# rogeliorjr/DyCON_Paper_Replication

Hardware: AMD Instinct MI355X
Metric: train volumes/sec (96^3 patch) (higher is better)
Workload: dtype bf16

## Files before the change

### dycon_paper_replication_amd/_lib.py

```python
from __future__ import annotations

import ctypes as C
import os

_HERE = os.path.dirname(os.path.abspath(__file__))
LIB_PATH = os.environ.get("DYCON_LIB", os.path.join(_HERE, "libdycon_hip.so"))

F32, BF16 = 0, 1
CONV_1X1, CONV_K3, CONV_K2S2 = 0, 1, 2

P, I, L, F, Z, U64 = C.c_void_p, C.c_int, C.c_longlong, C.c_float, C.c_size_t, C.c_uint64

SIGNATURES = {
    "dycon_version": (I, []),
    "dycon_last_error": (C.c_char_p, []),
    "dycon_bfrag_bytes": (Z, [I, I, I, I]),
    "dycon_pack_bfrag": (I, [P, P, I, I, I, I, I, L, L, L, L, I, P]),
    "dycon_pack_batch": (I, [P, I, I, P]),
    "dycon_pack_tcn": (I, [P, P, I, I, I, I, L, L, L, L, I, P]),
    "dycon_conv_gemm_workspace": (Z, [I, I, I, I, I, I, I, I, I]),
    "dycon_conv_gemm_plan": (I, [I, I, I, I, I, I, I, I, I, I, I, P]),
    "dycon_conv_kernel_name": (C.c_char_p, [I]),
    "dycon_conv_region_name": (C.c_char_p, [P]),
    "dycon_conv_gemm": (I, [P, P, P, P, I, I, I, I, I, I, I, I, I, I, I, P, Z, P]),
    "dycon_conv_gemm_splits": (I, [I, I, I, I, I, I, I, I, I]),
    "dycon_conv_gemm_ex": (I, [P, P, P, P, I, I, I, I, I, I, I, I, I, I, I, P, Z, I, P]),
    "dycon_conv_direct": (I, [P, I, P, P, P, I, I, I, I, I, I, I, I, I, P]),
    "dycon_conv_wgrad_workspace": (Z, [I, I, I, I, I, I, I]),
    "dycon_conv_wgrad_name": (C.c_char_p, [I, I, I, I, I, I, I, I, I]),
    "dycon_conv_wgrad": (I, [P, I, P, I, P, P, I, I, I, I, I, I, I, L, L, L, P, Z, P]),
    "dycon_colsum_workspace": (Z, [L, I]),
    "dycon_colsum": (I, [P, I, P, L, I, P, Z, P]),
    "dycon_norm_workspace": (Z, [I, L, I]),
    "dycon_norm_stats": (I, [P, I, I, L, I, I, F, P, P, P, F, P, Z, P]),
    "dycon_norm_fwd": (I, [P, P, I, I, L, I, I, F, P, P, P, I, P, P, P, P, F, P, Z, P]),
    "dycon_norm_fwd_is_fused": (I, [I, L, I, I]),
    "dycon_norm_fwd_slab": (I, [P, I, P, P, P, I, I, L, I, I, F, P, P, P, I, P, P, P]),
    "dycon_norm_apply": (I, [P, P, I, I, L, I, I, P, P, P, I, P, P, P]),
    "dycon_norm_bwd": (I, [P, I, P, P, I, I, L, I, I, P, P, P, I, P, P, P, P, Z, P]),
    "dycon_norm_bwd_ex": (I, [P, I, P, P, I, I, L, I, I, P, P, P, I, P, P, P, I, P, Z, P]),
    "dycon_norm_sum_dparams": (I, [P, I, I, P, P, P]),
# ... 243 lines not shown
```

### dycon_paper_replication_amd/csrc/conv.hip

```cpp
#include <stdlib.h>

#include "common.h"

typedef float f32x4 __attribute__((ext_vector_type(4)));
typedef __bf16 bf16x8 __attribute__((ext_vector_type(8)));

template <typename T> struct Frag;
template <> struct Frag<float> { static constexpr int G = 4, KC = 16; };
template <> struct Frag<bf16> { static constexpr int G = 8, KC = 32; };

__device__ __forceinline__ void mma(f32x4& acc, const Vec16<float>& a, const Vec16<float>& b) {
    acc = __builtin_amdgcn_mfma_f32_16x16x4f32(a.v.x, b.v.x, acc, 0, 0, 0);
    acc = __builtin_amdgcn_mfma_f32_16x16x4f32(a.v.y, b.v.y, acc, 0, 0, 0);
    acc = __builtin_amdgcn_mfma_f32_16x16x4f32(a.v.z, b.v.z, acc, 0, 0, 0);
    acc = __builtin_amdgcn_mfma_f32_16x16x4f32(a.v.w, b.v.w, acc, 0, 0, 0);
}
__device__ __forceinline__ void mma(f32x4& acc, const Vec16<bf16>& a, const Vec16<bf16>& b) {
    acc = __builtin_amdgcn_mfma_f32_16x16x32_bf16(__builtin_bit_cast(bf16x8, a.v), __builtin_bit_cast(bf16x8, b.v),
                                                  acc, 0, 0, 0);
}

template <int MODE> __device__ __forceinline__ int n_taps() { return MODE == DYCON_CONV_K3 ? 27 : MODE == DYCON_CONV_K2S2 ? 8 : 1; }

template <int MODE>
// ... 86 lines not shown
            if (++c == jb.Cin) { c = 0; ++t; }
        }
        if (jb.kind == 0) {
            uint4 o;
            o.x = (unsigned)f32_to_bf16_bits(v[0]) | ((unsigned)f32_to_bf16_bits(v[1]) << 16);
            o.y = (unsigned)f32_to_bf16_bits(v[2]) | ((unsigned)f32_to_bf16_bits(v[3]) << 16);
            o.z = (unsigned)f32_to_bf16_bits(v[4]) | ((unsigned)f32_to_bf16_bits(v[5]) << 16);
            o.w = (unsigned)f32_to_bf16_bits(v[6]) | ((unsigned)f32_to_bf16_bits(v[7]) << 16);
            reinterpret_cast<uint4*>(jb.out)[pi] = o;
        } else {
            reinterpret_cast<float4*>(jb.out)[pi] = make_float4(v[0], v[1], v[2], v[3]);
        }
    }
}

constexpr int NTB = 4;

template <typename T, int MODE, bool SCATTER>
__global__ __launch_bounds__(256) void conv_gemm_kernel(const T* __restrict__ X, const T* __restrict__ Wf,
                                                        const float* __restrict__ bias, T* __restrict__ Y, int B, int Di,
                                                        int Hi, int Wi, int Cin, int Do, int Ho, int Wo, int N, int Cout,
                                                        int NT, int nKC, int accumulate, float* __restrict__ slab,
                                                        int kc_per_split, int span_major = 0) {
    constexpr int G = Frag<T>::G, KC = Frag<T>::KC;
    const int lane = threadIdx.x & 63, wave = threadIdx.x >> 6;
    const int r = lane & 15, kg = lane >> 4;
    const long long M = (long long)B * Do * Ho * Wo;
    const long long m = (long long)blockIdx.x * 64 + wave * 16 + r;
    const bool mvalid = m < M;
    int xo, yo, zo, bo;
    {
        long long q = mvalid ? m : 0;
// ... 89 lines not shown
                                 2 * ox + (tap & 1);
            off = ov * Cout + co;
        } else {
            off = mo * N + n0;
        }
        Vec16<T> o = ld16(Ot + row * OS + pc * VN);
        if (accumulate) {
            const Vec16<T> old = ld16(Y + off);
#pragma unroll
            for (int k = 0; k < VN; ++k) o.set(k, o.get(k) + old.get(k));
        }
        st16(Y + off, o);
    }
}

constexpr int CT_BM = 64, CT_BN = 128, CT_AS = 40;
constexpr int CT_OS = CT_BN + 4;

template <int KS2>
__global__ __launch_bounds__(256, KS2 == 1 ? 4 : 3) void conv_k3_tile_kernel(const bf16* __restrict__ X, const bf16* __restrict__ Wf,
                                                           const float* __restrict__ bias, bf16* __restrict__ Y,
                                                           float* __restrict__ slab, int B, int D, int H, int W, int Cin, int N,
                                                           int NT, int nKC, int kc_per_split, int accumulate, int span_major = 0) {
    constexpr int A_ELEMS = CT_BM * CT_AS, B_ELEMS = 8 * 64 * 8;
    constexpr int KLOOP_BYTES = 2 * KS2 * (A_ELEMS + B_ELEMS) * 2, EPI_BYTES = CT_BM * CT_OS * 4;
    __shared__ __attribute__((aligned(16))) unsigned char lds_raw[KLOOP_BYTES > EPI_BYTES ? KLOOP_BYTES : EPI_BYTES];
    unsigned short (*As)[KS2][A_ELEMS] = reinterpret_cast<unsigned short (*)[KS2][A_ELEMS]>(lds_raw);
    unsigned short (*Bs)[KS2][B_ELEMS] = reinterpret_cast<unsigned short (*)[KS2][B_ELEMS]>(lds_raw + 2 * KS2 * A_ELEMS * 2);
    const int lane = threadIdx.x & 63, wave = threadIdx.x >> 6;
    const int r = lane & 15, kg = lane >> 4;
    const int wm = wave >> 1, wn = wave & 1;
// ... 172 lines not shown
            const int hz = hv / 36, hy = (hv / 6) % 6, hx = hv % 6;
            const int zi = z0 + hz - 1, yi = y0 + hy - 1, xi = x0 + hx - 1;
            v[i] = make_uint4(0, 0, 0, 0);
            if (p < PIECES && (unsigned)zi < (unsigned)D && (unsigned)yi < (unsigned)H && (unsigned)xi < (unsigned)W)
                v[i] = *reinterpret_cast<const uint4*>(xb + (((long long)zi * H + yi) * W + xi) * CH_CIN + sl * 8);
        }
#pragma unroll
        for (int i = 0; i < PER; ++i) {
            const int p = tid + i * 64 * CH_NW, hv = p >> 4, sl = p & 15;
            const int hy = (hv / 6) % 6, hx = hv % 6;
            if (p < PIECES) *reinterpret_cast<uint4*>(lds + hv * 256 + ((sl ^ (4 * (hy & 3) + (hx & 3))) * 16)) = v[i];
        }
    }

    auto load_b = [&](int kc, uint4 (&bf)[NJ]) {
        const uint4* p = reinterpret_cast<const uint4*>(Wf + ((long long)kc * NT + nt0 + cg * NJ) * 512) + lane;
#pragma unroll
        for (int j = 0; j < NJ; ++j) bf[j] = p[j * 64];
    };
    f32x4 acc[4][NJ];
#pragma unroll
    for (int m = 0; m < 4; ++m)
#pragma unroll
        for (int j = 0; j < NJ; ++j) acc[m][j] = f32x4{0.f, 0.f, 0.f, 0.f};
    auto compute = [&](int kc, const uint4 (&bf)[NJ]) {
        const int t = kc >> 2, kq = kc & 3;
        const int dz = t / 9, dy = (t / 3) % 3, dx = t % 3;
        const int hy = ry + dy, hx = rx + dx;
        const int slot = (4 * kq + kg) ^ (4 * (hy & 3) + (hx & 3));
        const unsigned char* ap = lds + ((dz * CH_H + hy) * CH_H + hx) * 256 + slot * 16;
        bf16x8 a[4];
// ... 2091 lines not shown
        pack_bfrag_kernel<T><<<grid, 256, 0, stream>>>(w, (T*)out, Tn, Cin, N, N0, s_t, s_c, s_n1, s_n0, flip_taps, NT, total);
    });
    DYCON_LAUNCH_CHECK();
    return DYCON_OK;
}

extern "C" int dycon_pack_tcn(const float* w, float* out, int T, int Cin, int N, int N0, long long s_t, long long s_c,
                              long long s_n1, long long s_n0, int flip_taps, dycon_stream_t stream) {
    DYCON_REQUIRE(w && out && T > 0 && Cin > 0 && N > 0 && N0 > 0, "pack_tcn: bad arguments");
    const long long total = (long long)T * Cin * N;
    pack_tcn_kernel<<<cdiv(total, 256), 256, 0, stream>>>(w, out, T, Cin, N, N0, s_t, s_c, s_n1, s_n0, flip_taps, total);
    DYCON_LAUNCH_CHECK();
    return DYCON_OK;
}

struct SplitK { int splits, kc_per_split; };
static SplitK splitk_plan(int dtype, int mode, int scatter, long long M, int N, int Cin) {
    const int KC = dtype == DYCON_BF16 ? 32 : 16;
    const int Tn = mode == DYCON_CONV_K3 ? 27 : mode == DYCON_CONV_K2S2 ? 8 : 1;
    const int nKC = (Tn * Cin + KC - 1) / KC;
    const long long wgs = ((M + 63) / 64) * (((N + 15) / 16 + NTB - 1) / NTB);
    SplitK p{1, nKC};
    if (scatter || wgs >= 512 || nKC < 16) return p;
    long long s = (1024 + wgs - 1) / wgs;
    if (s > nKC / 6) s = nKC / 6;
    if (s < 2) return p;
    p.kc_per_split = (int)((nKC + s - 1) / s);
    p.splits = (nKC + p.kc_per_split - 1) / p.kc_per_split;
    return p;
}
static SplitK conv_tile_plan(long long M, int N, int Cin) {
    constexpr long long target_wgs = 512;
    const int nKC = 27 * Cin / 32;
    const long long wgs = ((M + CT_BM - 1) / CT_BM) * (N / CT_BN);
    SplitK p{1, nKC};
    if (wgs >= 384) return p;
    long long s = target_wgs / wgs;
    if (s > nKC / 8) s = nKC / 8;
    if (s < 2) return p;
    p.kc_per_split = (int)((nKC + s - 1) / s);
    if (Cin % 64 == 0) p.kc_per_split = (p.kc_per_split + 1) & ~1;
    p.splits = (nKC + p.kc_per_split - 1) / p.kc_per_split;
    return p;
}

constexpr long long CONV_LDS_MIN_VOXELS = 13824;
static bool conv_first_layer(int dtype, int mode, int scatter, int Di, int Hi, int Wi, int Cin, int Cout) {
    return dtype == DYCON_BF16 && mode == DYCON_CONV_K3 && !scatter && Cin == 1 && (Cout == 16 || Cout == 32 || Cout == 64) &&
           (long long)Di * Hi * Wi >= CONV_LDS_MIN_VOXELS;
}
struct ConvRefusal { const char* fmt; int arg; };
static ConvRefusal conv_refusal(int dtype, int mode, int scatter, int B, int Di, int Hi, int Wi, int Cin, int N, int Cout) {
    if (!(B > 0 && Di > 0 && Hi > 0 && Wi > 0 && Cin > 0 && N > 0 && Cout > 0)) return {"conv_gemm: bad shape", 0};
    if (mode < 0 || mode > 2) return {"conv_gemm: bad mode %d", mode};
    if (!conv_first_layer(dtype, mode, scatter, Di, Hi, Wi, Cin, Cout) && Cin % (dtype == DYCON_BF16 ? 8 : 4) != 0)
        return {"conv_gemm: Cin=%d not a multiple of the fragment width", Cin};
    if (N % 16 != 0) return {"conv_gemm: N=%d not a multiple of 16 (use dycon_conv_direct)", N};
    if (scatter && !(mode == DYCON_CONV_1X1 && N == 8 * Cout)) return {"conv_gemm: scatter needs mode 1x1 and N == 8*Cout", 0};
    if (!scatter && N != Cout) return {"conv_gemm: N must equal Cout without scatter", 0};
// ... 559 lines not shown
```

### dycon_paper_replication_amd/engine.py

```python
from __future__ import annotations

from collections import OrderedDict
from typing import Dict, Optional

import torch

from . import ops
from ._lib import CONV_1X1, CONV_C1, CONV_K2S2, CONV_K3, CONV_W_CHUNK16

UNET_FILTERS = (16, 32, 64, 128, 256)
VNET_NORMS = ("groupnorm", "instancenorm", "batchnorm", "none")


def _projection_spec(spec, c_in):
    spec["projection.0.weight"] = (512, c_in, 1, 1, 1)
    spec["projection.0.bias"] = (512,)
    spec["projection.1.weight"] = (512,)
    spec["projection.1.bias"] = (512,)
    spec["projection.3.weight"] = (256, 512, 1, 1, 1)
    spec["projection.3.bias"] = (256,)
    spec["projection.4.weight"] = (256,)
    spec["projection.4.bias"] = (256,)


# ... 147 lines not shown
        self.use_aspp = net_type == "unet_3D" and "aspp.conv1.weight" in params
        self._aspp_plans = {}
        self._jobs_split, self._pack_event = False, None
        self.on_param_grads = None
        self.wgrad_stream = None
        self.wgrad_stream2 = None
        self._wg_flip = 0
        self.feat_stream = None
        self.mark = None
        self.Gs = {}
        self._head_range = (0, 0)
        self._wws = {}
        self.fuse_finish = False
        self.conv_stats = False
        self.conv_stats96 = False
        self._stat_parts = {}
        self._deferred = {}
        self._pending_dparams = []
        self.tape = []
        self.G = {}

    def params_changed(self):
        self.gen += 1

    def _pk(self, key, kind, w, T, Cin, N, N0, s_t, s_c, s_n1, s_n0, flip=False):
        hit = self._packed.get(key)
        if hit is not None and hit[0] == self.gen:
            return hit[1]
        buf = hit[1] if hit is not None else None
        if kind == "frag":
            buf = ops.pack_bfrag(w, self.dtype, T, Cin, N, N0, s_t, s_c, s_n1, s_n0, flip, out=buf)
            code = 0 if self.dtype == torch.bfloat16 else 1
# ... 94 lines not shown
    def _peek(self, t):
        g = self.G.get(id(t))
        if g is not None:
            self._sync_to(id(t), g)
        return g

    def _put(self, t, g):
        self.G[id(t)] = g
        if self.feat_stream is not None:
            self.Gs[id(t)] = ops.cur_stream()

    def _give(self, t, g):
        cur = self._peek(t)
        self._put(t, g if cur is None else ops.add(cur, g))

    def _conv(self, name, x, kind, need_gx=True, out_dtype=None, norm_groups=0):
        w, b = self.p[name + ".weight"], self.p[name + ".bias"]
        dtype = self.dtype
        if kind == "deconv":
            Cin, Cout = w.shape[0], w.shape[1]
        else:
            Cout, Cin = w.shape[0], w.shape[1]
        T = {"k3": 27, "k2s2": 8, "deconv": 8, "1x1": 1}[kind]
        mode = {"k3": CONV_K3, "k2s2": CONV_K2S2, "deconv": CONV_1X1, "1x1": CONV_1X1}[kind]
        gq = 8 if dtype == torch.bfloat16 else 4
        skinny = (Cin % gq != 0) or (Cout % 16 != 0)
        out_dtype = out_dtype or dtype
        plan = ops.conv_plan_for(x, mode, Cout, Cout) if kind == "k3" and out_dtype == dtype else None
        first_lds = plan is not None and plan.family == CONV_C1

        def conv_with_stats(wf, want):
# ... 11 lines not shown
                y = ops.conv_gemm(x, wf, b, CONV_K3, Cout, Cout)
        elif skinny:
            assert kind in ("k3", "1x1"), "skinny path only for the first conv and the 1x1 heads"
            wt = self._pk((name, "tcn"), "tcn", w, T, Cin, Cout, Cout, 1, T, 0, Cin * T)
            y = ops.conv_direct(x, wt, b, mode, Cout, out_dtype)
        elif kind == "deconv":
            wf = self._pk((name, "f"), "frag", w, 1, Cin, 8 * Cout, Cout, 0, Cout * 8, 1, 8)
            y = ops.conv_gemm(x, wf, b, CONV_1X1, 8 * Cout, Cout, scatter=True)
        elif plan is not None and plan.weights == CONV_W_CHUNK16:
            wf = self._pk_chunked16((name, "f48"), w, 3, Cout, 1, 27, Cin * 27)
            y = ops.conv_gemm(x, wf, b, mode, Cout, Cout)
        else:
            wf = self._pk((name, "f"), "frag", w, T, Cin, Cout, Cout, 1, T, 0, Cin * T)
            Vo = (x.shape[1] * x.shape[2] * x.shape[3]) // (8 if kind == "k2s2" else 1)
            want_stats = self.conv_stats96 if (Cin, Cout) == (16, 16) else self.conv_stats
            y = conv_with_stats(wf, want_stats and kind == "k3" and out_dtype == dtype and dtype == torch.bfloat16)
            if y is None and (norm_groups and self.fuse_finish and dtype == torch.bfloat16 and out_dtype == dtype
                              and ops.norm_fwd_is_fused(x, Vo, Cout, norm_groups)):
                y, dc = ops.conv_gemm(x, wf, b, mode, Cout, Cout, defer_finish=True)
                if dc is not None:
                    self._deferred[id(y)] = dc
            elif y is None:
                y = ops.conv_gemm(x, wf, b, mode, Cout, Cout)

        if self.recording:
            def wgrad(gy):
                gw, gb = self.g[name + ".weight"], self.g[name + ".bias"]
                wkey = (name, tuple(x.shape[:4]))
                ws = self._wws.get(wkey)
                if kind == "deconv":
                    if ws is None:
# ... 89 lines not shown
            if self.recording:
                def bwd_relu():
                    gy = self._take(y)
                    if skip is not None:
                        self._give(skip, gy)
                    self._give(z, ops.relu_bwd(z, gy, chan_scale))
                self.tape.append(bwd_relu)
            return y
        Nb, V, C, G, gamma, beta, rm, rv = self._norm_site(prefix, z, kind)
        if kind == "bn" and not training:
            stats = self._eval_stats(rm, rv)
            y = ops.norm_apply(z, stats, Nb, V, C, G, gamma, beta, relu, skip, chan_scale=chan_scale)
        elif id(z) in self._stat_parts and kind in ("gn", "in"):
            part, chunks = self._stat_parts.pop(id(z))
            y, stats = ops.norm_fwd_parts(z, part, chunks, Nb, V, C, G, gamma, beta, relu, skip, chan_scale)
        elif id(z) in self._deferred:
            y, stats = ops.norm_fwd_slab(z, self._deferred.pop(id(z)), Nb, V, C, G, gamma, beta, relu, skip, chan_scale)
        else:
            upd = kind == "bn" and training and self.update_bn
            y, stats = ops.norm_fwd(z, Nb, V, C, G, gamma, beta, relu, skip, chan_scale, 1e-5, rm if upd else None,
                                    rv if upd else None, 0.1)
            if upd:
                self._count_batch(prefix)
        if self.recording:
            def bwd():
                gy = self._take(y)
                if skip is not None:
                    self._give(skip, gy)
                dg = self.g[prefix + ".weight"] if gamma is not None else None
                db = self.g[prefix + ".bias"] if beta is not None else None
# ... 278 lines not shown

    def _fuses_first_block(self, x, nk, training):
        w1 = self.p["block_one.conv.0.weight"]
        return (self.dtype == torch.bfloat16 and nk != "none" and not (nk == "bn" and not training)
                and w1.shape[0] == 16 and w1.shape[1] == 1 and x.shape[0] <= 16)

    def _vnet(self, x, training):
        nk = {"groupnorm": "gn", "instancenorm": "in", "batchnorm": "bn", "none": "none"}[self.normalization]
        st = 2 if nk == "none" else 3

        def ngroups(t, conv):
            return 16 if nk == "gn" else (self.p[conv + ".weight"].shape[0] if nk == "in" else 0)

        def block(name, t, n, first=False, drop=None):
            for i in range(n):
                t = self._conv(f"{name}.conv.{st * i}", t, "k3", need_gx=not (first and i == 0), norm_groups=ngroups(t, f"{name}.conv.{st * i}"))
                cs = None
                if drop is not None and i == n - 1:
                    cs = self._channel_scale(t.shape[0], t.shape[-1], drop[0], 0.5, drop[1], t.device)
                t = self._norm(f"{name}.conv.{st * i + 1}", t, nk, chan_scale=cs, training=training)
            return t

        def down(name, t):
            return self._norm(f"{name}.conv.1", self._conv(f"{name}.conv.0", t, "k2s2", norm_groups=ngroups(t, f"{name}.conv.0")), nk,
                              training=training)

        def up(name, t, skip):
            return self._norm(f"{name}.conv.1", self._conv(f"{name}.conv.0", t, "deconv"), nk, skip=skip, training=training)

        if self._fuses_first_block(x, nk, training):
            x1 = self._first_block("block_one", x, nk, training)
        else:
            x1 = block("block_one", x, 1, first=True)
        self.pack_ready()
        x2 = block("block_two", down("block_one_dw", x1), 2)
        x3 = block("block_three", down("block_two_dw", x2), 3)
        x4 = block("block_four", down("block_three_dw", x3), 3)
        x5 = block("block_five", down("block_four_dw", x4), 3, drop=("drop5", 0))
        x5_ready = self._mark_ready()
        u = up("block_five_up", x5, x4)
# ... 59 lines not shown
        if want_sdf:
            rec, self.recording = self.recording, False
            sdf = ops.tanh(self._conv("final", u1, "1x1", out_dtype=torch.float32))
            self.recording = rec
        return logits, feats, sdf

    def forward(self, x, training=True, record=True, dropout: Optional[DropoutSpec] = None, update_bn=True,
                want_sdf=False):
        assert x.dim() == 5 and x.is_contiguous()
        self.recording = bool(record)
        self.update_bn = update_bn
        self.dropout = dropout or DropoutSpec("off")
        self.tape, self.G = [], {}
        self._deferred = {}
        self._stat_parts = {}
        if x.dtype != self.dtype:
            x = ops.cast(x, self.dtype)
        if self.net_type == "vnet":
            logits, feats, sdf = self._vnet(x, training)
            if want_sdf:
                sdf = ops.tanh(logits)
        else:
            logits, feats, sdf = self._unet(x, training, want_sdf)
        self._out = (logits, feats)
        return logits, feats, sdf

    def backward(self, g_logits: Optional[torch.Tensor], g_feats: Optional[torch.Tensor]):
        logits, feats = self._out
        if g_logits is None:
            g_logits = torch.zeros_like(logits)
# ... 35 lines not shown
```

### dycon_paper_replication_amd/ops.py

```python
from __future__ import annotations

import collections
import ctypes
import functools
from typing import Optional

import torch

from . import _lib
from ._lib import BF16, CONV_1X1, CONV_K2S2, CONV_K3, F32, call, query

_DT = {torch.float32: F32, torch.bfloat16: BF16}


def dt(t: torch.Tensor) -> int:
    try:
        return _DT[t.dtype]
    except KeyError:
        raise TypeError(f"unsupported dtype {t.dtype}: the HIP path stores fp32 or bf16") from None


_STREAMS = []


# ... 259 lines not shown

def conv_stats_chunks(x, Cin, Cout):
    return conv_plan_for(x, CONV_K3, Cout, Cout).chunks


def conv_gemm_stats(x, wfrag, bias, Cout, chunks):
    B, D, H, W, Cin = x.shape
    y = torch.empty((B, D, H, W, Cout), dtype=x.dtype, device=x.device)
    part = torch.empty(B * chunks * Cout * 2, dtype=torch.float32, device=x.device)
    with _Region(conv_plan_for(x, CONV_K3, Cout, Cout).name, (x.numel() + y.numel()) * _es(x) + 27 * Cin * Cout * _es(x),
                 2 * (y.numel() // Cout) * 27 * Cin * Cout):
        call("dycon_conv_gemm_stats", _p(x), _p(wfrag), _p(bias), _p(y), dt(x), B, D, H, W, Cin, Cout, _p(part), part.numel() * 4, _s())
    return y, part


def conv_direct(x, w_tcn, bias, mode, N, out_dtype, out=None, accumulate=False):
    B, D, H, W, Cin = x.shape
    if out is None:
        assert not accumulate
        shape = (B, D // 2, H // 2, W // 2, N) if mode == CONV_K2S2 else (B, D, H, W, N)
        out = torch.empty(shape, dtype=out_dtype, device=x.device)
    taps = _TAPS[mode]
    with _Region("conv_direct", x.numel() * _es(x) + out.numel() * _es(out), 2 * (out.numel() // N) * taps * Cin * N):
        call("dycon_conv_direct", _p(x), dt(x), _p(w_tcn), _p(bias), _p(out), dt(out), mode, int(accumulate),
             B, D, H, W, Cin, N, _s())
    return out


def conv_wgrad_workspace(x, gy, mode):
    B, D, H, W, Cin = x.shape
# ... 632 lines not shown
```

### include/dycon_hip.h

```cpp
#ifndef DYCON_HIP_H
#define DYCON_HIP_H

#include <stddef.h>
#include <stdint.h>

#ifdef __cplusplus
extern "C" {
#endif

typedef struct ihipStream_t* dycon_stream_t;

#define DYCON_F32 0
#define DYCON_BF16 1

#define DYCON_OK 0
#define DYCON_ERR_INVALID (-22)
#define DYCON_ERR_LAUNCH (-5)

#define DYCON_CONV_1X1 0
#define DYCON_CONV_K3 1
#define DYCON_CONV_K2S2 2

int dycon_version(void);
const char* dycon_last_error(void);
// ... 23 lines not shown
} dycon_conv_plan_t;
int dycon_conv_gemm_plan(int dtype, int mode, int scatter, int accumulate, int B, int Di, int Hi, int Wi, int Cin, int N,
                         int Cout, dycon_conv_plan_t* plan);
const char* dycon_conv_kernel_name(int family);
const char* dycon_conv_region_name(const dycon_conv_plan_t* plan);
size_t dycon_conv_gemm_workspace(int dtype, int mode, int scatter, int B, int Di, int Hi, int Wi,
                                 int Cin, int N);
int dycon_conv_gemm(const void* x, const void* wfrag, const float* bias, void* y, int dtype,
                    int mode, int scatter, int accumulate, int B, int Di, int Hi, int Wi, int Cin,
                    int N, int Cout, float* workspace, size_t ws_bytes, dycon_stream_t stream);
int dycon_conv_gemm_splits(int dtype, int mode, int scatter, int B, int Di, int Hi, int Wi, int Cin, int N);
int dycon_conv_gemm_ex(const void* x, const void* wfrag, const float* bias, void* y, int dtype,
                       int mode, int scatter, int accumulate, int B, int Di, int Hi, int Wi, int Cin,
                       int N, int Cout, float* workspace, size_t ws_bytes, int defer_finish,
                       dycon_stream_t stream);
int dycon_conv_direct(const void* x, int x_dtype, const float* w_tcn, const float* bias, void* y,
                      int y_dtype, int mode, int accumulate, int B, int Di, int Hi, int Wi, int Cin,
                      int N, dycon_stream_t stream);

size_t dycon_conv_wgrad_workspace(int mode, int B, int Di, int Hi, int Wi, int Cin, int Cout);
const char* dycon_conv_wgrad_name(int x_dtype, int g_dtype, int mode, int B, int Di, int Hi, int Wi, int Cin, int Cout);
int dycon_conv_wgrad(const void* x, int x_dtype, const void* gy, int g_dtype, float* dw, float* dbias,
                     int mode, int B, int Di, int Hi, int Wi, int Cin, int Cout, long long s_t,
                     long long s_c, long long s_n, float* workspace, size_t ws_bytes,
                     dycon_stream_t stream);

size_t dycon_colsum_workspace(long long rows, int C);
int dycon_colsum(const void* x, int dtype, float* out, long long rows, int C, float* workspace,
                 size_t ws_bytes, dycon_stream_t stream);

// ... 313 lines not shown
```

Baseline: 923.4.

## Fuse bottleneck k3 conv with GroupNorm in a per-sample LDS-resident kernel

Adds a kernel that processes one sample per workgroup for small spatial volumes (at most 256 output voxels). It stages the whole input sample in LDS and runs the 3x3x3 convolution with MFMA, then applies GroupNorm, affine, ReLU and channel scaling in the same kernel. The engine routes bottleneck k3 conv+GN pairs through this path when the shape is accepted, which removes the separate stats and normalize launches and their extra HBM round trips. The cost is a low-occupancy launch (one block of 512 threads per CU) with large LDS use, and a grid of only B x Cout/16 blocks.

Result: no change. 923.2 (-0.0%).

```diff
diff --git a/dycon_paper_replication_amd/_lib.py b/dycon_paper_replication_amd/_lib.py
--- a/dycon_paper_replication_amd/_lib.py
+++ b/dycon_paper_replication_amd/_lib.py
@@ -25,6 +25,9 @@
     "dycon_conv_gemm": (I, [P, P, P, P, I, I, I, I, I, I, I, I, I, I, I, P, Z, P]),
     "dycon_conv_gemm_splits": (I, [I, I, I, I, I, I, I, I, I]),
     "dycon_conv_gemm_ex": (I, [P, P, P, P, I, I, I, I, I, I, I, I, I, I, I, P, Z, I, P]),
+    "dycon_conv_sample_ok": (I, [I, I, I, I, I, I, I, I, I]),
+    "dycon_conv_sample": (I, [P, P, P, P, I, I, I, I, I, I, I, I, I, P]),
+    "dycon_conv_norm_fwd": (I, [P, P, P, P, P, I, I, I, I, I, I, I, I, I, F, P, P, P, I, P, P, P]),
     "dycon_conv_direct": (I, [P, I, P, P, P, I, I, I, I, I, I, I, I, I, P]),
     "dycon_conv_wgrad_workspace": (Z, [I, I, I, I, I, I, I]),
     "dycon_conv_wgrad_name": (C.c_char_p, [I, I, I, I, I, I, I, I, I]),
diff --git a/dycon_paper_replication_amd/csrc/bottleneck.hip b/dycon_paper_replication_amd/csrc/bottleneck.hip
--- /dev/null
+++ b/dycon_paper_replication_amd/csrc/bottleneck.hip
@@ -0,0 +1,317 @@
+#include "common.h"
+#include "conv_plan.h"
+#include "norm_fused.h"
+
+typedef float f32x4 __attribute__((ext_vector_type(4)));
+typedef __bf16 bf16x8 __attribute__((ext_vector_type(8)));
+
+constexpr int SG_NW = 8;
+constexpr int SG_MAXV = 32 * SG_NW;
+constexpr int SG_DEPTH = 4;
+constexpr int SG_TILE_BYTES = SG_MAXV * 16 * 2;
+constexpr int SG_LDS_MAX = 160 * 1024 - 1024;
+
+template <int MODE, bool NORM, int CPT>
+__global__ __launch_bounds__(64 * SG_NW, 1) void conv_sample_group_kernel(
+    const bf16* __restrict__ X, const bf16* __restrict__ Wf, const float* __restrict__ bias, bf16* __restrict__ Z, bf16* __restrict__ Y,
+    int Di, int Hi, int Wi, int Cin, int N, int nKC, int kc_per_split, int accumulate, int G, float eps, float* __restrict__ stats,
+    const float* __restrict__ gamma, const float* __restrict__ beta, int relu, const bf16* __restrict__ skip,
+    const float* __restrict__ chan_scale) {
+    extern __shared__ __attribute__((aligned(16))) unsigned char lds[];
+    __shared__ float sm[4 * 2 * 16];
+    unsigned short* zt = reinterpret_cast<unsigned short*>(lds);
+    unsigned char* img = lds + SG_TILE_BYTES;
+    const int tid = threadIdx.x, lane = tid & 63, wave = tid >> 6;
+    const int r = lane & 15, kg = lane >> 4;
+    const int b = blockIdx.x, nt = blockIdx.y, NT = N >> 4;
+    const int Do = MODE == DYCON_CONV_K2S2 ? Di >> 1 : Di, Ho = MODE == DYCON_CONV_K2S2 ? Hi >> 1 : Hi, Wo = MODE == DYCON_CONV_K2S2 ? Wi >> 1 : Wi;
+    const int V = Do * Ho * Wo;
+    const int cpt = Cin >> 5;
+    const int nslots = Cin >> 3, pitch = Cin * 2;
+    const bool wide = (nslots & 15) == 0;
+    auto swz = [&](int v) { return wide ? (v & 15) : ((v >> 1) & 7); };
+
+    uint4 b0[CPT > 0 ? CPT : 1], b1[CPT > 0 ? CPT : 1];
+    auto load_tap_b = [&](int t, uint4 (&bb)[CPT > 0 ? CPT : 1]) {
+#pragma unroll
+        for (int q = 0; q < CPT; ++q) bb[q] = *bfrag_bf16(Wf, t * CPT + q, NT, nt, lane);
+    };
+    if (MODE == DYCON_CONV_K3) {
+        if (CPT > 0) load_tap_b(0, b0);
+        const uint4* xs = reinterpret_cast<const uint4*>(X + (long long)b * V * Cin);
+        const int pieces = (V + 1) * nslots, real = V * nslots;
+        constexpr int SU = 16;
+        for (int p0 = 0; p0 < pieces; p0 += SU * 64 * SG_NW) {
+            uint4 v[SU];
+#pragma unroll
+            for (int u = 0; u < SU; ++u) {
+                const int p = p0 + u * 64 * SG_NW + tid;
+                v[u] = make_uint4(0, 0, 0, 0);
+                if (p < real) v[u] = xs[p];
+            }
+#pragma unroll
+            for (int u = 0; u < SU; ++u) {
+                const int p = p0 + u * 64 * SG_NW + tid;
+                if (p < pieces) {
+                    const int vox = p / nslots, s = p - vox * nslots;
+                    *reinterpret_cast<uint4*>(img + vox * pitch + ((s ^ swz(vox)) << 4)) = v[u];
+                }
+            }
+        }
+    }
+
+    int mrow[2];
+    unsigned vmask[2] = {0u, 0u};
+    long long gbase[2] = {0, 0};
+    bool mvalid[2];
+#pragma unroll
+    for (int j = 0; j < 2; ++j) {
+        const int m = (2 * wave + j) * 16 + r;
+        mvalid[j] = m < V;
+        mrow[j] = mvalid[j] ? m : V - 1;
+        const int x = mrow[j] % Wo, y = (mrow[j] / Wo) % Ho, z = mrow[j] / (Wo * Ho);
+        if (MODE == DYCON_CONV_K3) {
+            for (int t = 0; t < 27; ++t) {
+                const int zi = z + t / 9 - 1, yi = y + (t / 3) % 3 - 1, xi = x + t % 3 - 1;
+                if (mvalid[j] && (unsigned)zi < (unsigned)Di && (unsigned)yi < (unsigned)Hi && (unsigned)xi < (unsigned)Wi) vmask[j] |= 1u << t;
+            }
+        } else {
+            gbase[j] = ((((long long)b * Di + 2 * z) * Hi + 2 * y) * Wi + 2 * x) * Cin + 8 * kg;
+        }
+    }
+
+    const unsigned char* arow[2] = {img, img};
+    int axor[2] = {0, 0};
+    bool ain[2] = {false, false};
+    auto set_tap = [&](int t) {
+        const int dz = t / 9, dy = (t / 3) % 3, dx = t % 3;
+        const int off = ((dz - 1) * Hi + (dy - 1)) * Wi + (dx - 1);
+#pragma unroll
+        for (int j = 0; j < 2; ++j) {
+            ain[j] = ((vmask[j] >> t) & 1u) != 0;
+            const int sv = ain[j] ? mrow[j] + off : mrow[j];
+            arow[j] = img + sv * pitch;
+            axor[j] = swz(sv);
+        }
+    };
+    auto load_a = [&](int kc, uint4 (&a)[2]) {
+        const int t = kc / cpt, kq = kc - t * cpt;
+        const long long off = ((long long)((t >> 2) * Hi + ((t >> 1) & 1)) * Wi + (t & 1)) * Cin + 32 * kq;
+#pragma unroll
+        for (int j = 0; j < 2; ++j) {
+            a[j] = *reinterpret_cast<const uint4*>(X + gbase[j] + off);
+            if (!mvalid[j]) a[j] = make_uint4(0, 0, 0, 0);
+        }
+    };
+
+    const int col = nt * 16 + r;
+    const float bv = bias ? bias[col] : 0.f;
+    float warm = 0.f;
+    if (NORM) {
+        if (gamma) warm += gamma[col];
+        if (beta) warm += beta[col];
+        if (chan_scale) warm += chan_scale[(long long)b * N + col];
+    }
+    f32x4 acc[2], run[2];
+#pragma unroll
+    for (int j = 0; j < 2; ++j) { acc[j] = f32x4{0.f, 0.f, 0.f, 0.f}; run[j] = f32x4{bv, bv, bv, bv}; }
+
+    if constexpr (MODE == DYCON_CONV_K3 && CPT > 0) {
+        __syncthreads();
+        if (2 * wave * 16 < V) {
+            const unsigned char* zrow = img + V * pitch;
+            int kend = min(kc_per_split, nKC);
+            auto tap = [&](int t, const uint4 (&bb)[CPT]) {
+                const int dz = t / 9, dy = (t / 3) % 3, dx = t % 3;
+                const int off = ((dz - 1) * Hi + (dy - 1)) * Wi + (dx - 1);
+                uint4 av[2][CPT];
+#pragma unroll
+                for (int j = 0; j < 2; ++j) {
+                    const bool in = ((vmask[j] >> t) & 1u) != 0;
+                    const int sv = mrow[j] + off;
+                    const unsigned char* ar = in ? img + sv * pitch : zrow;
+                    const int ax = in ? swz(sv) : 0;
+#pragma unroll
+                    for (int q = 0; q < CPT; ++q) av[j][q] = *reinterpret_cast<const uint4*>(ar + (((4 * q + kg) ^ ax) << 4));
+                }
+#pragma unroll
+                for (int q = 0; q < CPT; ++q) {
+                    const bf16x8 bb8 = __builtin_bit_cast(bf16x8, bb[q]);
+#pragma unroll
+                    for (int j = 0; j < 2; ++j)
+                        acc[j] = __builtin_amdgcn_mfma_f32_16x16x32_bf16(__builtin_bit_cast(bf16x8, av[j][q]), bb8, acc[j], 0, 0, 0);
+                    if ((q & 1) && t * CPT + q + 1 == kend) {
+#pragma unroll
+                        for (int j = 0; j < 2; ++j) { run[j] += acc[j]; acc[j] = f32x4{0.f, 0.f, 0.f, 0.f}; }
+                        kend = min(kend + kc_per_split, nKC);
+                    }
+                }
+            };
+            for (int t = 0; t < 27; t += 2) {
+                if (t + 1 < 27) load_tap_b(t + 1, b1);
+                tap(t, b0);
+                if (t + 1 < 27) {
+                    if (t + 2 < 27) load_tap_b(t + 2, b0);
+                    tap(t + 1, b1);
+                }
+            }
+        }
+    } else {
+        uint4 bq[SG_DEPTH], aq[SG_DEPTH][2];
+#pragma unroll
+        for (int u = 0; u < SG_DEPTH; ++u) {
+            if (u < nKC) {
+                bq[u] = *bfrag_bf16(Wf, u, NT, nt, lane);
+                if (MODE == DYCON_CONV_K2S2) load_a(u, aq[u]);
+            }
+        }
+        if (MODE == DYCON_CONV_K3) {
+            set_tap(0);
+            __syncthreads();
+        }
+        int t = 0, kq = 0, kend = min(kc_per_split, nKC);
+        for (int kc0 = 0; kc0 < nKC; kc0 += SG_DEPTH) {
+#pragma unroll
+            for (int u = 0; u < SG_DEPTH; ++u) {
+                const int kc = kc0 + u;
+                if (kc < nKC) {
+                    bf16x8 a[2];
+#pragma unroll
+                    for (int j = 0; j < 2; ++j) {
+                        if (MODE == DYCON_CONV_K3) {
+                            uint4 v = *reinterpret_cast<const uint4*>(arow[j] + (((4 * kq + kg) ^ axor[j]) << 4));
+                            if (!ain[j]) v = make_uint4(0, 0, 0, 0);
+                            a[j] = __builtin_bit_cast(bf16x8, v);
+                        } else {
+                            a[j] = __builtin_bit_cast(bf16x8, aq[u][j]);
+                        }
+                    }
+                    const bf16x8 bb = __builtin_bit_cast(bf16x8, bq[u]);
+#pragma unroll
+                    for (int j = 0; j < 2; ++j) acc[j] = __builtin_amdgcn_mfma_f32_16x16x32_bf16(a[j], bb, acc[j], 0, 0, 0);
+                    if (kc + SG_DEPTH < nKC) {
+                        bq[u] = *bfrag_bf16(Wf, kc + SG_DEPTH, NT, nt, lane);
+                        if (MODE == DYCON_CONV_K2S2) load_a(kc + SG_DEPTH, aq[u]);
+                    }
+                    if (MODE == DYCON_CONV_K3) {
+                        if (++kq == cpt) { kq = 0; ++t; set_tap(min(t, 26)); }
+                    }
+                    if (kc + 1 == kend) {
+#pragma unroll
+                        for (int j = 0; j < 2; ++j) { run[j] += acc[j]; acc[j] = f32x4{0.f, 0.f, 0.f, 0.f}; }
+                        kend = min(kend + kc_per_split, nKC);
+                    }
+                }
+            }
+        }
+    }
+
+    bf16* out = NORM ? Z : Y;
+#pragma unroll
+    for (int j = 0; j < 2; ++j)
+#pragma unroll
+        for (int i = 0; i < 4; ++i) {
+            const int row = (2 * wave + j) * 16 + 4 * kg + i;
+            float v = run[j][i];
+            if (!NORM && accumulate && row < V) v += ldf(out + ((long long)b * V + row) * N + col);
+            zt[row * 16 + r] = f32_to_bf16_bits(v);
+        }
+    __syncthreads();
+    if (!NORM) {
+        const int row = tid >> 1, pc = tid & 1;
+        if (row < V)
+            *reinterpret_cast<uint4*>(out + ((long long)b * V + row) * N + nt * 16 + pc * 8) = *reinterpret_cast<const uint4*>(zt + row * 16 + pc * 8);
+        return;
+    }
+    asm volatile("" ::"v"(warm));
+    Vec16<bf16> xr[1][2];
+    const int vc = tid < V ? tid : V - 1;
+#pragma unroll
+    for (int q = 0; q < 2; ++q) {
+        xr[0][q].v = *reinterpret_cast<const uint4*>(zt + vc * 16 + q * 8);
+        if (out && tid < V) st16(out + ((long long)b * V + tid) * N + nt * 16 + q * 8, xr[0][q]);
+    }
+    norm_fused_tail<bf16, 16, 16, 1>(xr, Y, b, nt * 16, (long long)V, N, G, eps, stats, gamma, beta, relu, skip, chan_scale, nullptr, nullptr, 0.f,
+                                     false, sm);
+}
+
+static const char* sample_refusal(int dtype, int mode, int B, int D, int H, int W, int Cin, int Cout, int G) {
+    if (dtype != DYCON_BF16) return "bf16 storage only";
+    if (mode != DYCON_CONV_K3 && mode != DYCON_CONV_K2S2) return "mode must be k3 or k2s2";
+    if (!(B > 0 && B <= 65535 && D > 0 && H > 0 && W > 0 && Cin > 0 && Cout > 0 && G >= 0)) return "bad shape";
+    if (mode == DYCON_CONV_K2S2 && (D % 2 || H % 2 || W % 2)) return "k2s2 needs even dims";
+    const long long V = mode == DYCON_CONV_K2S2 ? (long long)(D / 2) * (H / 2) * (W / 2) : (long long)D * H * W;
+    if (V <= 0 || V > SG_MAXV) return "more than 256 output voxels per sample";
+    if (Cin % 64 != 0) return "Cin must be a multiple of 64";
+    if (Cout % 16 != 0 || (mode == DYCON_CONV_K3 && Cout % CT_BN != 0)) return "Cout must be a multiple of 16 (k3: of 128)";
+    if (mode == DYCON_CONV_K3 && SG_TILE_BYTES + (V + 1) * Cin * 2 > SG_LDS_MAX) return "the sample (and a row of zeros) does not fit LDS";
+    if (G > 0 && (Cout % G != 0 || Cout / G != 16)) return "GroupNorm with 16 channels per group only";
+    return nullptr;
+}
+
+template <int MODE, bool NORM, int CPT>
+static int sample_launch_cpt(const void* x, const void* wfrag, const float* bias, void* z, void* y, int B, int D, int H, int W, int Cin, int N,
+                  int accumulate, int G, float eps, float* stats, const float* gamma, const float* beta, int relu, const void* skip,
+                  const float* chan_scale, dycon_stream_t stream) {
+    const long long V = MODE == DYCON_CONV_K2S2 ? (long long)(D / 2) * (H / 2) * (W / 2) : (long long)D * H * W;
+    const int nKC = (MODE == DYCON_CONV_K3 ? 27 : 8) * Cin / 32;
+    const SplitK sk = MODE == DYCON_CONV_K3 ? conv_tile_plan(B * V, N, Cin) : splitk_plan(DYCON_BF16, MODE, 0, B * V, N, Cin);
+    const size_t lds = SG_TILE_BYTES + (MODE == DYCON_CONV_K3 ? (size_t)(V + 1) * Cin * 2 : 0);
+    static size_t reserved = 0;
+    if (lds > 48 * 1024 && lds > reserved) {
+        if (hipFuncSetAttribute((const void*)conv_sample_group_kernel<MODE, NORM, CPT>, hipFuncAttributeMaxDynamicSharedMemorySize, (int)lds) != hipSuccess) {
+            dycon_set_error("conv_sample: cannot reserve %zu bytes of LDS", lds);
+            return DYCON_ERR_LAUNCH;
+        }
+        reserved = lds;
+    }
+    conv_sample_group_kernel<MODE, NORM, CPT><<<dim3(B, N / 16), 64 * SG_NW, lds, stream>>>(
+        (const bf16*)x, (const bf16*)wfrag, bias, (bf16*)z, (bf16*)y, D, H, W, Cin, N, nKC, sk.kc_per_split, accumulate, G, eps, stats, gamma,
+        beta, relu, (const bf16*)skip, chan_scale);
+    DYCON_LAUNCH_CHECK();
+    return DYCON_OK;
+}
+
+template <int MODE, bool NORM>
+static int sample_launch(const void* x, const void* wfrag, const float* bias, void* z, void* y, int B, int D, int H, int W, int Cin, int N,
+                         int accumulate, int G, float eps, float* stats, const float* gamma, const float* beta, int relu, const void* skip,
+                         const float* chan_scale, dycon_stream_t stream) {
+#define DYCON_SG(CPTV) sample_launch_cpt<MODE, NORM, CPTV>(x, wfrag, bias, z, y, B, D, H, W, Cin, N, accumulate, G, eps, stats, gamma, beta, relu, skip, chan_scale, stream)
+    if constexpr (MODE == DYCON_CONV_K3) {
+        if (Cin == 256) return DYCON_SG(8);
+        if (Cin == 128) return DYCON_SG(4);
+    }
+    return DYCON_SG(0);
+#undef DYCON_SG
+}
+
+extern "C" int dycon_conv_sample_ok(int dtype, int mode, int B, int D, int H, int W, int Cin, int Cout, int G) {
+    return sample_refusal(dtype, mode, B, D, H, W, Cin, Cout, G) ? 0 : 1;
+}
+
+extern "C" int dycon_conv_sample(const void* x, const void* wfrag, const float* bias, void* y, int dtype, int mode, int accumulate, int B,
+                                 int D, int H, int W, int Cin, int Cout, dycon_stream_t stream) {
+    DYCON_REQUIRE(x && wfrag && y, "conv_sample: null pointer");
+    const char* no = sample_refusal(dtype, mode, B, D, H, W, Cin, Cout, 0);
+    DYCON_REQUIRE(!no, "conv_sample: %s (ask dycon_conv_sample_ok)", no);
+    DYCON_REQUIRE(!(mode == DYCON_CONV_K2S2 && accumulate), "conv_sample: k2s2 does not accumulate");
+    if (mode == DYCON_CONV_K3)
+        return sample_launch<DYCON_CONV_K3, false>(x, wfrag, bias, nullptr, y, B, D, H, W, Cin, Cout, accumulate, 0, 0.f, nullptr, nullptr, nullptr,
+                                                   0, nullptr, nullptr, stream);
+    return sample_launch<DYCON_CONV_K2S2, false>(x, wfrag, bias, nullptr, y, B, D, H, W, Cin, Cout, 0, 0, 0.f, nullptr, nullptr, nullptr, 0, nullptr,
+                                                 nullptr, stream);
+}
+
+extern "C" int dycon_conv_norm_fwd(const void* x, const void* wfrag, const float* bias, void* z, void* y, int dtype, int mode, int B, int D,
+                                   int H, int W, int Cin, int Cout, int G, float eps, float* stats, const float* gamma, const float* beta,
+                                   int relu, const void* skip, const float* chan_scale, dycon_stream_t stream) {
+    DYCON_REQUIRE(x && wfrag && y && stats, "conv_norm_fwd: null pointer");
+    DYCON_REQUIRE(G > 0, "conv_norm_fwd: G=%d groups", G);
+    const char* no = sample_refusal(dtype, mode, B, D, H, W, Cin, Cout, G);
+    DYCON_REQUIRE(!no, "conv_norm_fwd: %s (ask dycon_conv_sample_ok)", no);
+    if (mode == DYCON_CONV_K3)
+        return sample_launch<DYCON_CONV_K3, true>(x, wfrag, bias, z, y, B, D, H, W, Cin, Cout, 0, G, eps, stats, gamma, beta, relu, skip, chan_scale,
+                                                  stream);
+    return sample_launch<DYCON_CONV_K2S2, true>(x, wfrag, bias, z, y, B, D, H, W, Cin, Cout, 0, G, eps, stats, gamma, beta, relu, skip, chan_scale,
+                                                stream);
+}
diff --git a/dycon_paper_replication_amd/csrc/conv.hip b/dycon_paper_replication_amd/csrc/conv.hip
--- a/dycon_paper_replication_amd/csrc/conv.hip
+++ b/dycon_paper_replication_amd/csrc/conv.hip
@@ -1,6 +1,7 @@
 #include <stdlib.h>
 
 #include "common.h"
+#include "conv_plan.h"
 
 typedef float f32x4 __attribute__((ext_vector_type(4)));
 typedef __bf16 bf16x8 __attribute__((ext_vector_type(8)));
@@ -124,8 +125,6 @@
     }
 }
 
-constexpr int NTB = 4;
-
 template <typename T, int MODE, bool SCATTER>
 __global__ __launch_bounds__(256) void conv_gemm_kernel(const T* __restrict__ X, const T* __restrict__ Wf,
                                                         const float* __restrict__ bias, T* __restrict__ Y, int B, int Di,
@@ -245,7 +244,7 @@
     }
 }
 
-constexpr int CT_BM = 64, CT_BN = 128, CT_AS = 40;
+constexpr int CT_AS = 40;
 constexpr int CT_OS = CT_BN + 4;
 
 template <int KS2>
@@ -448,7 +447,7 @@
     }
 
     auto load_b = [&](int kc, uint4 (&bf)[NJ]) {
-        const uint4* p = reinterpret_cast<const uint4*>(Wf + ((long long)kc * NT + nt0 + cg * NJ) * 512) + lane;
+        const uint4* p = bfrag_bf16(Wf, kc, NT, nt0 + cg * NJ, lane);
 #pragma unroll
         for (int j = 0; j < NJ; ++j) bf[j] = p[j * 64];
     };
@@ -2570,35 +2569,6 @@
     return DYCON_OK;
 }
 
-struct SplitK { int splits, kc_per_split; };
-static SplitK splitk_plan(int dtype, int mode, int scatter, long long M, int N, int Cin) {
-    const int KC = dtype == DYCON_BF16 ? 32 : 16;
-    const int Tn = mode == DYCON_CONV_K3 ? 27 : mode == DYCON_CONV_K2S2 ? 8 : 1;
-    const int nKC = (Tn * Cin + KC - 1) / KC;
-    const long long wgs = ((M + 63) / 64) * (((N + 15) / 16 + NTB - 1) / NTB);
-    SplitK p{1, nKC};
-    if (scatter || wgs >= 512 || nKC < 16) return p;
-    long long s = (1024 + wgs - 1) / wgs;
-    if (s > nKC / 6) s = nKC / 6;
-    if (s < 2) return p;
-    p.kc_per_split = (int)((nKC + s - 1) / s);
-    p.splits = (nKC + p.kc_per_split - 1) / p.kc_per_split;
-    return p;
-}
-static SplitK conv_tile_plan(long long M, int N, int Cin) {
-    constexpr long long target_wgs = 512;
-    const int nKC = 27 * Cin / 32;
-    const long long wgs = ((M + CT_BM - 1) / CT_BM) * (N / CT_BN);
-    SplitK p{1, nKC};
-    if (wgs >= 384) return p;
-    long long s = target_wgs / wgs;
-    if (s > nKC / 8) s = nKC / 8;
-    if (s < 2) return p;
-    p.kc_per_split = (int)((nKC + s - 1) / s);
-    if (Cin % 64 == 0) p.kc_per_split = (p.kc_per_split + 1) & ~1;
-    p.splits = (nKC + p.kc_per_split - 1) / p.kc_per_split;
-    return p;
-}
 
 constexpr long long CONV_LDS_MIN_VOXELS = 13824;
 static bool conv_first_layer(int dtype, int mode, int scatter, int Di, int Hi, int Wi, int Cin, int Cout) {
diff --git a/dycon_paper_replication_amd/csrc/conv_plan.h b/dycon_paper_replication_amd/csrc/conv_plan.h
--- /dev/null
+++ b/dycon_paper_replication_amd/csrc/conv_plan.h
@@ -0,0 +1,39 @@
+#pragma once
+#include "common.h"
+
+constexpr int NTB = 4;
+constexpr int CT_BM = 64, CT_BN = 128;
+
+struct SplitK { int splits, kc_per_split; };
+static inline SplitK splitk_plan(int dtype, int mode, int scatter, long long M, int N, int Cin) {
+    const int KC = dtype == DYCON_BF16 ? 32 : 16;
+    const int Tn = mode == DYCON_CONV_K3 ? 27 : mode == DYCON_CONV_K2S2 ? 8 : 1;
+    const int nKC = (Tn * Cin + KC - 1) / KC;
+    const long long wgs = ((M + 63) / 64) * (((N + 15) / 16 + NTB - 1) / NTB);
+    SplitK p{1, nKC};
+    if (scatter || wgs >= 512 || nKC < 16) return p;
+    long long s = (1024 + wgs - 1) / wgs;
+    if (s > nKC / 6) s = nKC / 6;
+    if (s < 2) return p;
+    p.kc_per_split = (int)((nKC + s - 1) / s);
+    p.splits = (nKC + p.kc_per_split - 1) / p.kc_per_split;
+    return p;
+}
+static inline SplitK conv_tile_plan(long long M, int N, int Cin) {
+    constexpr long long target_wgs = 512;
+    const int nKC = 27 * Cin / 32;
+    const long long wgs = ((M + CT_BM - 1) / CT_BM) * (N / CT_BN);
+    SplitK p{1, nKC};
+    if (wgs >= 384) return p;
+    long long s = target_wgs / wgs;
+    if (s > nKC / 8) s = nKC / 8;
+    if (s < 2) return p;
+    p.kc_per_split = (int)((nKC + s - 1) / s);
+    if (Cin % 64 == 0) p.kc_per_split = (p.kc_per_split + 1) & ~1;
+    p.splits = (nKC + p.kc_per_split - 1) / p.kc_per_split;
+    return p;
+}
+
+__device__ __forceinline__ const uint4* bfrag_bf16(const bf16* __restrict__ Wf, int kc, int NT, int nt, int lane) {
+    return reinterpret_cast<const uint4*>(Wf + ((long long)kc * NT + nt) * 512) + lane;
+}
diff --git a/dycon_paper_replication_amd/csrc/norm_fused.h b/dycon_paper_replication_amd/csrc/norm_fused.h
--- /dev/null
+++ b/dycon_paper_replication_amd/csrc/norm_fused.h
@@ -0,0 +1,98 @@
+#pragma once
+#include "common.h"
+
+template <int NV>
+__device__ __forceinline__ void block_reduce_vec4(float (&v)[NV], float* sm ) {
+    const int lane = threadIdx.x & 63, wv = threadIdx.x >> 6;
+#pragma unroll
+    for (int k = 0; k < NV; ++k) v[k] = wave_sum(v[k]);
+    __syncthreads();
+    if (lane == 0 && wv < 4) {
+#pragma unroll
+        for (int k = 0; k < NV; ++k) sm[wv * NV + k] = v[k];
+    }
+    __syncthreads();
+#pragma unroll
+    for (int k = 0; k < NV; ++k) v[k] = sm[k] + sm[NV + k] + sm[2 * NV + k] + sm[3 * NV + k];
+}
+
+template <typename T, int SPAN, int CPG, int NF_ROWS>
+__device__ __forceinline__ void norm_fused_tail(const Vec16<T> (&xr)[NF_ROWS][SPAN / Vec16<T>::N], T* __restrict__ Y, int n, int c0,
+                                                long long V, int C, int G, float eps, float* __restrict__ stats,
+                                                const float* __restrict__ gamma, const float* __restrict__ beta, int relu,
+                                                const T* __restrict__ skip, const float* __restrict__ chan_scale, float* running_mean,
+                                                float* running_var, float momentum, bool one_sample, float* sm ) {
+    constexpr int VN = Vec16<T>::N, NVEC = SPAN / VN;
+    constexpr int cpg = CPG;
+    float acc[2 * SPAN];
+#pragma unroll
+    for (int k = 0; k < 2 * SPAN; ++k) acc[k] = 0.f;
+#pragma unroll
+    for (int i = 0; i < NF_ROWS; ++i) {
+        const bool ok = (long long)threadIdx.x + 256 * i < V;
+#pragma unroll
+        for (int q = 0; q < NVEC; ++q)
+#pragma unroll
+            for (int k = 0; k < VN; ++k) { const float f = ok ? xr[i][q].get(k) : 0.f; acc[q * VN + k] += f; acc[SPAN + q * VN + k] += f * f; }
+    }
+    block_reduce_vec4<2 * SPAN>(acc, sm);
+    float sc[SPAN], sh[SPAN], cs[SPAN];
+    const double cnt = (double)V * cpg;
+#pragma unroll
+    for (int k = 0; k < SPAN; ++k) {
+        const int gl = k / cpg;
+        double s0 = 0.0, s1 = 0.0;
+#pragma unroll
+        for (int j = 0; j < SPAN; ++j)
+            if (j / cpg == gl) { s0 += acc[j]; s1 += acc[SPAN + j]; }
+        const double mean = s0 / cnt;
+        double var = s1 / cnt - mean * mean;
+        if (var < 0.0) var = 0.0;
+        const float rstd = (float)(1.0 / sqrt(var + (double)eps));
+        const int c = c0 + k;
+        const float gm = gamma ? gamma[c] : 1.f, bt = beta ? beta[c] : 0.f;
+        sc[k] = rstd * gm;
+        sh[k] = bt - (float)mean * rstd * gm;
+        cs[k] = chan_scale ? chan_scale[(long long)n * C + c] : 1.f;
+        if (threadIdx.x == 0 && (k % cpg) == 0) {
+            const int g = c / cpg;
+            stats[((long long)n * G + g) * 2] = (float)mean;
+            stats[((long long)n * G + g) * 2 + 1] = rstd;
+            if (running_mean && one_sample && G == C) {
+                running_mean[g] = (1.f - momentum) * running_mean[g] + momentum * (float)mean;
+                const double unb = cnt > 1.0 ? var * cnt / (cnt - 1.0) : var;
+                running_var[g] = (1.f - momentum) * running_var[g] + momentum * (float)unb;
+            }
+        }
+    }
+    T* yp = Y + (long long)n * V * C + c0;
+    const T* sp = skip ? skip + (long long)n * V * C + c0 : nullptr;
+    Vec16<T> sr[NF_ROWS][NVEC];
+    if (sp) {
+#pragma unroll
+        for (int i = 0; i < NF_ROWS; ++i) {
+            const long long v = threadIdx.x + 256 * i, vc = v < V ? v : V - 1;
+#pragma unroll
+            for (int q = 0; q < NVEC; ++q) sr[i][q] = ld16(sp + vc * C + q * VN);
+        }
+    }
+#pragma unroll
+    for (int i = 0; i < NF_ROWS; ++i) {
+        const long long v = threadIdx.x + 256 * i;
+        if (v < V) {
+#pragma unroll
+            for (int q = 0; q < NVEC; ++q) {
+                Vec16<T> y;
+#pragma unroll
+                for (int k = 0; k < VN; ++k) {
+                    float f = xr[i][q].get(k) * sc[q * VN + k] + sh[q * VN + k];
+                    if (relu) f = f < 0.f ? 0.f : f;
+                    f *= cs[q * VN + k];
+                    if (sp) f += sr[i][q].get(k);
+                    y.set(k, f);
+                }
+                st16(yp + v * C + q * VN, y);
+            }
+        }
+    }
+}
diff --git a/dycon_paper_replication_amd/engine.py b/dycon_paper_replication_amd/engine.py
--- a/dycon_paper_replication_amd/engine.py
+++ b/dycon_paper_replication_amd/engine.py
@@ -185,8 +185,10 @@
         self.fuse_finish = False
         self.conv_stats = False
         self.conv_stats96 = False
+        self.fuse_bottleneck = True
         self._stat_parts = {}
         self._deferred = {}
+        self._normed = {}
         self._pending_dparams = []
         self.tape = []
         self.G = {}
@@ -311,7 +313,16 @@
         cur = self._peek(t)
         self._put(t, g if cur is None else ops.add(cur, g))
 
-    def _conv(self, name, x, kind, need_gx=True, out_dtype=None, norm_groups=0):
+    def _conv_norm(self, cname, nname, x, kind, nk, need_gx=True, norm_groups=0, chan_scale=None, training=True):
+        fused = None
+        if self.fuse_bottleneck and nk == "gn" and self.dtype == torch.bfloat16 and kind == "k3":
+            Cout = self.p[cname + ".weight"].shape[0]
+            if ops.conv_sample_ok(x, CONV_K3, Cout, 16):
+                fused = (16, self.p[nname + ".weight"], self.p[nname + ".bias"], chan_scale)
+        z = self._conv(cname, x, kind, need_gx=need_gx, norm_groups=norm_groups, fused_norm=fused)
+        return self._norm(nname, z, nk, chan_scale=chan_scale, training=training)
+
+    def _conv(self, name, x, kind, need_gx=True, out_dtype=None, norm_groups=0, fused_norm=None):
         w, b = self.p[name + ".weight"], self.p[name + ".bias"]
         dtype = self.dtype
         if kind == "deconv":
@@ -353,7 +364,14 @@
             wf = self._pk((name, "f"), "frag", w, T, Cin, Cout, Cout, 1, T, 0, Cin * T)
             Vo = (x.shape[1] * x.shape[2] * x.shape[3]) // (8 if kind == "k2s2" else 1)
             want_stats = self.conv_stats96 if (Cin, Cout) == (16, 16) else self.conv_stats
-            y = conv_with_stats(wf, want_stats and kind == "k3" and out_dtype == dtype and dtype == torch.bfloat16)
+            if fused_norm is not None:
+                G, gamma, beta, cs = fused_norm
+                y, yn, stats = ops.conv_norm_fwd(x, wf, b, mode, Cout, G, gamma, beta, True, None, cs, keep_z=self.recording)
+                if y is None:
+                    y = yn
+                self._normed[id(y)] = (yn, stats)
+            else:
+                y = conv_with_stats(wf, want_stats and kind == "k3" and out_dtype == dtype and dtype == torch.bfloat16)
             if y is None and (norm_groups and self.fuse_finish and dtype == torch.bfloat16 and out_dtype == dtype
                               and ops.norm_fwd_is_fused(x, Vo, Cout, norm_groups)):
                 y, dc = ops.conv_gemm(x, wf, b, mode, Cout, Cout, defer_finish=True)
@@ -473,6 +491,8 @@
         elif id(z) in self._stat_parts and kind in ("gn", "in"):
             part, chunks = self._stat_parts.pop(id(z))
             y, stats = ops.norm_fwd_parts(z, part, chunks, Nb, V, C, G, gamma, beta, relu, skip, chan_scale)
+        elif id(z) in self._normed:
+            y, stats = self._normed.pop(id(z))
         elif id(z) in self._deferred:
             y, stats = ops.norm_fwd_slab(z, self._deferred.pop(id(z)), Nb, V, C, G, gamma, beta, relu, skip, chan_scale)
         else:
@@ -781,16 +801,17 @@
 
         def block(name, t, n, first=False, drop=None):
             for i in range(n):
-                t = self._conv(f"{name}.conv.{st * i}", t, "k3", need_gx=not (first and i == 0), norm_groups=ngroups(t, f"{name}.conv.{st * i}"))
+                cname = f"{name}.conv.{st * i}"
                 cs = None
                 if drop is not None and i == n - 1:
-                    cs = self._channel_scale(t.shape[0], t.shape[-1], drop[0], 0.5, drop[1], t.device)
-                t = self._norm(f"{name}.conv.{st * i + 1}", t, nk, chan_scale=cs, training=training)
+                    cs = self._channel_scale(t.shape[0], self.p[cname + ".weight"].shape[0], drop[0], 0.5, drop[1], t.device)
+                t = self._conv_norm(cname, f"{name}.conv.{st * i + 1}", t, "k3", nk, need_gx=not (first and i == 0),
+                                    norm_groups=ngroups(t, cname), chan_scale=cs, training=training)
             return t
 
         def down(name, t):
-            return self._norm(f"{name}.conv.1", self._conv(f"{name}.conv.0", t, "k2s2", norm_groups=ngroups(t, f"{name}.conv.0")), nk,
-                              training=training)
+            return self._conv_norm(f"{name}.conv.0", f"{name}.conv.1", t, "k2s2", nk, norm_groups=ngroups(t, f"{name}.conv.0"),
+                                   training=training)
 
         def up(name, t, skip):
             return self._norm(f"{name}.conv.1", self._conv(f"{name}.conv.0", t, "deconv"), nk, skip=skip, training=training)
@@ -880,6 +901,7 @@
         self.tape, self.G = [], {}
         self._deferred = {}
         self._stat_parts = {}
+        self._normed = {}
         if x.dtype != self.dtype:
             x = ops.cast(x, self.dtype)
         if self.net_type == "vnet":
diff --git a/dycon_paper_replication_amd/ops.py b/dycon_paper_replication_amd/ops.py
--- a/dycon_paper_replication_amd/ops.py
+++ b/dycon_paper_replication_amd/ops.py
@@ -297,6 +297,41 @@
     return y, part
 
 
+def conv_sample_ok(x, mode, Cout, G=0):
+    B, D, H, W, Cin = x.shape
+    return bool(query("dycon_conv_sample_ok", dt(x), mode, B, D, H, W, Cin, Cout, G))
+
+
+def _sample_out(x, mode, Cout):
+    B, D, H, W, _ = x.shape
+    shape = (B, D // 2, H // 2, W // 2, Cout) if mode == CONV_K2S2 else (B, D, H, W, Cout)
+    return torch.empty(shape, dtype=x.dtype, device=x.device)
+
+
+def conv_sample(x, wfrag, bias, mode, Cout, out=None, accumulate=False):
+    B, D, H, W, Cin = x.shape
+    if out is None:
+        assert not accumulate
+        out = _sample_out(x, mode, Cout)
+    with _Region("conv_sample_group", (x.numel() + out.numel() * (2 if accumulate else 1)) * _es(x) + _TAPS[mode] * Cin * Cout * _es(x),
+                 2 * (out.numel() // Cout) * _TAPS[mode] * Cin * Cout):
+        call("dycon_conv_sample", _p(x), _p(wfrag), _p(bias), _p(out), dt(x), mode, int(accumulate), B, D, H, W, Cin, Cout, _s())
+    return out
+
+
+def conv_norm_fwd(x, wfrag, bias, mode, Cout, G, gamma=None, beta=None, relu=True, skip=None, chan_scale=None, eps=1e-5, keep_z=True):
+    B, D, H, W, Cin = x.shape
+    y = _sample_out(x, mode, Cout)
+    z = torch.empty_like(y) if keep_z else None
+    stats = torch.empty(B * G * 2, dtype=torch.float32, device=x.device)
+    nout = y.numel() * ((2 if keep_z else 1) + (1 if skip is not None else 0))
+    with _Region("conv_sample_group", (x.numel() + nout) * _es(x) + _TAPS[mode] * Cin * Cout * _es(x),
+                 2 * (y.numel() // Cout) * _TAPS[mode] * Cin * Cout):
+        call("dycon_conv_norm_fwd", _p(x), _p(wfrag), _p(bias), _p(z), _p(y), dt(x), mode, B, D, H, W, Cin, Cout, G, eps, _p(stats),
+             _p(gamma), _p(beta), int(relu), _p(skip), _p(chan_scale), _s())
+    return z, y, stats
+
+
 def conv_direct(x, w_tcn, bias, mode, N, out_dtype, out=None, accumulate=False):
     B, D, H, W, Cin = x.shape
     if out is None:
diff --git a/include/dycon_hip.h b/include/dycon_hip.h
--- a/include/dycon_hip.h
+++ b/include/dycon_hip.h
@@ -61,6 +61,13 @@
                        int mode, int scatter, int accumulate, int B, int Di, int Hi, int Wi, int Cin,
                        int N, int Cout, float* workspace, size_t ws_bytes, int defer_finish,
                        dycon_stream_t stream);
+int dycon_conv_sample_ok(int dtype, int mode, int B, int D, int H, int W, int Cin, int Cout, int G);
+int dycon_conv_sample(const void* x, const void* wfrag, const float* bias, void* y, int dtype, int mode,
+                      int accumulate, int B, int D, int H, int W, int Cin, int Cout, dycon_stream_t stream);
+int dycon_conv_norm_fwd(const void* x, const void* wfrag, const float* bias, void* z, void* y, int dtype,
+                        int mode, int B, int D, int H, int W, int Cin, int Cout, int G, float eps, float* stats,
+                        const float* gamma, const float* beta, int relu, const void* skip,
+                        const float* chan_scale, dycon_stream_t stream);
 int dycon_conv_direct(const void* x, int x_dtype, const float* w_tcn, const float* bias, void* y,
                       int y_dtype, int mode, int accumulate, int B, int Di, int Hi, int Wi, int Cin,
                       int N, dycon_stream_t stream);
```
